# xuhaocuhk/TilinGNN

Measured on AMD Instinct MI355X. Metric: scored tile-nodes/sec (GNN forward), higher is better.
Workload: dtype f32; 1 GPU; TilinGNN.forward on a seeded banded super-graph: 100000 nodes / 1000000 adjacency edges / 1250000 collision edges per GPU, tile_count 2, T=13 edge types, width 32, depth 20, train-mode BatchNorm, graph prep included; n_nodes=100000, n_adj_edges=1000000, n_col_edges=1250000, parallelism=single GPU

## Files before the change

### tilingnn_amd/csrc/graph_prep.hip

```cpp
#include <atomic>
#include <chrono>
#include <mutex>
#include <vector>

#include "tgnn_common.h"

namespace tgnn {

constexpr int kScanThreads = 256;
constexpr int kScanItems = 8;
constexpr int kScanTile = kScanThreads * kScanItems;

__device__ __forceinline__ int wave_inclusive_scan(int v) {
    const int lane = threadIdx.x & 63;
#pragma unroll
    for (int d = 1; d < 64; d <<= 1) {
        int t = __shfl_up(v, d, 64);
        if (lane >= d) v += t;
    }
    return v;
}

__global__ __launch_bounds__(kScanThreads) void scan_tiles_kernel(const int *in, int *out,
                                                                  int *__restrict__ block_sums, int64_t n) {
// ... 894 lines not shown
                        e0 = rpA[row];
                        e1 = rpA[row + 1];
                    }
                    for (int e = e0; e < e1; e += 8) {
                        int ty[8];
#pragma unroll
                        for (int u = 0; u < 8; ++u) ty[u] = e + u < e1 ? A.adj_type[e + u] : -1;
#pragma unroll
                        for (int u = 0; u < 8; ++u)
                            if (ty[u] >= 0) cnt[tid * ld + ty[u]]++;
                    }
                }
                __syncthreads();
                if (act)
                    for (int t = i; t < n_types; t += 16) {
                        int m = 0;
                        for (int r = 0; r < 16; ++r) m = max(m, cnt[(k * 16 + r) * ld + t]);
                        maxm[k * kMaxColTypes + t] = m;
                    }
                __syncthreads();
                if (act && i == 0) {
                    int acc = 0;
                    for (int t = 0; t < n_types; ++t) {
                        base[k * (kMaxColTypes + 1) + t] = acc;
                        acc += maxm[k * kMaxColTypes + t];
                    }
                    base[k * (kMaxColTypes + 1) + n_types] = acc;
                    if (!fill && tile < nt16) g_tile_cols[tile] = acc + 1;
                }
                __syncthreads();
                if (fill && act && tile < nt16) {
                    const int64_t c0 = tile_ptr[tile];
                    const int n_edge_cols = base[k * (kMaxColTypes + 1) + n_types];
                    for (int c = 0; c < n_edge_cols; ++c) A.col_slot_src[(c0 + c) * 16 + i] = -1;
                    for (int t = i; t < n_types; t += 16) {
                        const int m = maxm[k * kMaxColTypes + t];
                        for (int r = 0; r < m; ++r)
                            A.col_meta[c0 + base[k * (kMaxColTypes + 1) + t] + r] = t | (r == 0 ? 1 << 8 : 0) | (r == m - 1 ? 1 << 9 : 0);
                    }
                    const int deg = e1 - e0;
                    A.col_slot_src[(c0 + n_edge_cols) * 16 + i] = row < n ? __float_as_int((float)(deg > 0 ? deg : 1)) : -1;
                    if (i == 0) A.col_meta[c0 + n_edge_cols] = n_types | (1 << 8) | (1 << 9) | (1 << 10);
                    __builtin_amdgcn_fence(__ATOMIC_RELEASE, "wavefront");
                    __builtin_amdgcn_wave_barrier();
                    for (int t = 0; t < n_types; ++t) cnt[tid * ld + t] = 0;
                    for (int e = e0; e < e1; e += 8) {
                        int ty[8], sr[8];
#pragma unroll
                        for (int u = 0; u < 8; ++u) {
                            ty[u] = e + u < e1 ? A.adj_type[e + u] : -1;
                            sr[u] = e + u < e1 ? A.adj_src[e + u] : 0;
                        }
#pragma unroll
                        for (int u = 0; u < 8; ++u)
                            if (ty[u] >= 0) {
                                const int r = cnt[tid * ld + ty[u]]++;
                                A.col_slot_src[(c0 + base[k * (kMaxColTypes + 1) + ty[u]] + r) * 16 + i] = sr[u];
                            }
                    }
                }
                __syncthreads();
            }
            if (!fill) {
                small_prep_barrier(A.ctr, target, G);
                for (int t = tid; t <= nt16; t += NT) tile_ptr[t] = t < nt16 ? g_tile_cols[t] : 0;
                __syncthreads();
                small_block_scan(tile_ptr, nt16 + 1, wave_tot);
                if (blk == 0)
                    for (int t = tid; t <= nt16; t += NT) A.tile_col_ptr[t] = tile_ptr[t];
                __syncthreads();
            }
        }
    } else {
        small_prep_barrier(A.ctr, target, G);
    }
    TGNN_PT
    if (blk == 0 && tid == 0) {
        A.result[0] = n_types;
        A.result[1] = g_flags[0];
        A.result[2] = g_flags[1];
        A.result[3] = ec_valid;
        A.result[4] = maxdeg;
        A.result[5] = cols ? 1 : 0;
        A.result[6] = fallback ? 1 : 0;
        if (!kUnion && A.result_host) {
            const int w[7] = {n_types, g_flags[0], g_flags[1], ec_valid, maxdeg, cols ? 1 : 0, fallback ? 1 : 0};
#pragma unroll
            for (int k = 0; k < 7; ++k) __hip_atomic_store(A.result_host + k, w[k], __ATOMIC_RELAXED, __HIP_MEMORY_SCOPE_SYSTEM);
            for (int k = 7; k < 31; ++k) __hip_atomic_store(A.result_host + k, 0, __ATOMIC_RELAXED, __HIP_MEMORY_SCOPE_SYSTEM);
            __threadfence_system();
            __hip_atomic_store(A.result_host + 31, kPrepWordsMagic, __ATOMIC_RELEASE, __HIP_MEMORY_SCOPE_SYSTEM);
        }
    }
    if (kUnion && blk == 0 && tid >= 7 && tid < 32) A.result[tid] = 0;
    __syncthreads();
    if (tid == 0 && atomicAdd(&A.ctr[1], 1u) == (unsigned)G - 1) {
        __hip_atomic_store(&A.ctr[0], 0u, __ATOMIC_RELAXED, __HIP_MEMORY_SCOPE_AGENT);
        __hip_atomic_store(&A.ctr[1], 0u, __ATOMIC_RELAXED, __HIP_MEMORY_SCOPE_AGENT);
    }
}

__global__ __launch_bounds__(kSmallPrepThreads) void graph_prep_small_kernel(SmallPrepArgs A) {
    graph_prep_small_body<false>(A, (int)blockIdx.x, (int)gridDim.x);
}

__global__ __launch_bounds__(kSmallPrepThreads) void graph_prep_small_union_kernel(const SmallPrepArgs *__restrict__ tab,
                                                                                   const int *__restrict__ first_block, int n_layouts) {
    int lo = 0, hi = n_layouts;
    while (hi - lo > 1) {
        const int mid = (lo + hi) >> 1;
        if (first_block[mid] <= (int)blockIdx.x) lo = mid; else hi = mid;
    }
    const int j = __builtin_amdgcn_readfirstlane(lo);
    const int b0 = __builtin_amdgcn_readfirstlane(first_block[j]), b1 = __builtin_amdgcn_readfirstlane(first_block[j + 1]);
    const SmallPrepArgs *e = tab + j;
    SmallPrepArgs A;
    A.adj_ei = e->adj_ei; A.col_ei = e->col_ei; A.attr = e->attr;
    A.n = e->n; A.ea = e->ea; A.ec = e->ec; A.fe = e->fe; A.max_col_types = e->max_col_types;
    A.adj_rowptr = e->adj_rowptr; A.adj_src = e->adj_src; A.adj_eid = e->adj_eid; A.adj_type = e->adj_type;
    A.edge_type = e->edge_type; A.type_rep = e->type_rep;
    A.col_rowptr = e->col_rowptr; A.col_src = e->col_src; A.col_eid = e->col_eid;
    A.tile_col_ptr = e->tile_col_ptr; A.col_meta = e->col_meta; A.col_slot_src = e->col_slot_src;
    A.result_host = nullptr; A.tmp = e->tmp; A.result = e->result; A.ctr = e->ctr;
    graph_prep_small_body<true>(A, (int)blockIdx.x - b0, b1 - b0);
}

static inline unsigned grid_for(int64_t n, int threads = 256, int cap = 256 * 16) {
    int64_t g = (n + threads - 1) / threads;
    if (g < 1) g = 1;
    if (g > cap) g = cap;
    return (unsigned)g;
}

static inline uint32_t dedup_table_size(int64_t e) {
    uint64_t want = (uint64_t)(e > 512 ? e : 512) * 2;
    uint32_t cap = 1024;
    while (cap < want) cap <<= 1;
    return cap;
}


constexpr int kBkLogMax = 9, kBkRows = 1 << kBkLogMax, kBkMaxBuckets = 4096, kBkThreads = 1024;
constexpr int kBkCap = 15360;
constexpr int kBkCapHalf = 7168;
struct BkSet {
    const int64_t *ei;
    int64_t e;
    int drop_self;
    int *rowptr, *col_src, *col_eid, *err_flag;
    int *rec_eid, *rec_src;
    unsigned short *rec_row;
    int *total_out, *max_deg_out;
};
struct BkArgs {
    BkSet set[2];
    int64_t n, n_src;
    int nb, nblk;
    int lg;
    int cap;
    int cap_lds;
    int *hist;
    const int *tile_off;
    unsigned *scan_ticket;
};
__device__ __forceinline__ int bk_scanned(const BkArgs &A, int64_t i) {
    const int v = A.hist[i];
    return A.tile_off ? v + A.tile_off[i / kScanTile] : v;
}

__global__ __launch_bounds__(kBkThreads) void bk_hist_kernel(BkArgs A) {
    extern __shared__ int bk_h[];
    const BkSet S = A.set[blockIdx.y];
    const int tid = threadIdx.x, blk = blockIdx.x;
    for (int b = tid; b < A.nb; b += kBkThreads) bk_h[b] = 0;
    __syncthreads();
    const int64_t i0 = S.e * blk / A.nblk, i1 = S.e * (blk + 1) / A.nblk;
    for (int64_t i = i0 + tid; i < i1; i += kBkThreads) {
        const int64_t s = S.ei[i], d = S.ei[S.e + i];
        if (s < 0 || s >= A.n_src || d < 0 || d >= A.n) {
            if (S.err_flag) *S.err_flag = 1;
        } else if (!(S.drop_self && s == d)) {
            atomicAdd(&bk_h[d >> A.lg], 1);
        }
    }
    __syncthreads();
    for (int b = tid; b < A.nb; b += kBkThreads) A.hist[((int64_t)blockIdx.y * A.nb + b) * A.nblk + blk] = bk_h[b];
    if (blk == 0 && blockIdx.y == 1 && tid == 0) {
        A.hist[(int64_t)2 * A.nb * A.nblk] = 0;
        if (A.scan_ticket) *A.scan_ticket = 0u;
    }
}

constexpr int kBkChunk = kBkThreads * 8;
__global__ __launch_bounds__(kBkThreads) void bk_scatter_kernel(BkArgs A) {
    extern __shared__ int bk_h[];
    int *cur = bk_h, *lcnt = cur + A.nb, *lstart = lcnt + A.nb, *wtot = lstart + A.nb;
    int *l_eid = wtot + 16, *l_src = l_eid + kBkChunk;
    unsigned short *l_row = reinterpret_cast<unsigned short *>(l_src + kBkChunk), *l_bkt = l_row + kBkChunk;
    const BkSet S = A.set[blockIdx.y];
    const int tid = threadIdx.x, blk = blockIdx.x;
    const int base = bk_scanned(A, (int64_t)blockIdx.y * A.nb * A.nblk);
    for (int b = tid; b < A.nb; b += kBkThreads) cur[b] = bk_scanned(A, ((int64_t)blockIdx.y * A.nb + b) * A.nblk + blk) - base;
    const int64_t i0 = S.e * blk / A.nblk, i1 = S.e * (blk + 1) / A.nblk;
    const int per = (A.nb + kBkThreads - 1) / kBkThreads;
    for (int64_t c0 = i0; c0 < i1; c0 += kBkChunk) {
        for (int b = tid; b < A.nb; b += kBkThreads) lcnt[b] = 0;
        __syncthreads();
        int e_b[8], e_r[8], e_s[8], e_row[8];
#pragma unroll
        for (int u = 0; u < 8; ++u) {
            const int64_t i = c0 + tid + (int64_t)u * kBkThreads;
            e_b[u] = -1;
            if (i < i1) {
                const int64_t sv = S.ei[i], d = S.ei[S.e + i];
                if (!(sv < 0 || sv >= A.n_src || d < 0 || d >= A.n || (S.drop_self && sv == d))) {
                    e_b[u] = (int)(d >> A.lg);
                    e_row[u] = (int)(d & ((1 << A.lg) - 1));
                    e_s[u] = (int)sv;
                    e_r[u] = atomicAdd(&lcnt[e_b[u]], 1);
                }
            }
        }
        __syncthreads();
        {
            int mine = 0;
            for (int q = 0; q < per; ++q) {
                const int b = tid * per + q;
                mine += b < A.nb ? lcnt[b] : 0;
            }
            const int incl = wave_inclusive_scan(mine);
            if ((tid & 63) == 63) wtot[tid >> 6] = incl;
            __syncthreads();
            int run = incl - mine;
            for (int w = 0; w < (tid >> 6); ++w) run += wtot[w];
            for (int q = 0; q < per; ++q) {
                const int b = tid * per + q;
                if (b < A.nb) {
                    lstart[b] = run;
                    run += lcnt[b];
                }
            }
        }
        __syncthreads();
        int total = 0;
#pragma unroll
        for (int u = 0; u < 8; ++u)
            if (e_b[u] >= 0) {
                const int at = lstart[e_b[u]] + e_r[u];
                l_eid[at] = (int)(c0 + tid + (int64_t)u * kBkThreads);
                l_src[at] = e_s[u];
                l_row[at] = (unsigned short)e_row[u];
                l_bkt[at] = (unsigned short)e_b[u];
            }
        total = lstart[A.nb - 1] + lcnt[A.nb - 1];
        __syncthreads();
        for (int j = tid; j < total; j += kBkThreads) {
            const int b = l_bkt[j];
            const int g = cur[b] + (j - lstart[b]);
            S.rec_eid[g] = l_eid[j];
            S.rec_src[g] = l_src[j];
            S.rec_row[g] = l_row[j];
        }
        __syncthreads();
        for (int b = tid; b < A.nb; b += kBkThreads) cur[b] += lcnt[b];
    }
}

__global__ __launch_bounds__(kBkThreads) void bk_rows_kernel(BkArgs A) {
    extern __shared__ int bk_l[];
    const int rows = 1 << A.lg;
    int *cnt = bk_l, *off = bk_l + rows, *wtot = off + rows + 1, *key_s = wtot + 16, *val_s = key_s + A.cap_lds;
    unsigned short *row_s = reinterpret_cast<unsigned short *>(val_s + A.cap_lds);
    const BkSet S = A.set[blockIdx.y];
    const int tid = threadIdx.x, b = blockIdx.x;
    const int base = bk_scanned(A, (int64_t)blockIdx.y * A.nb * A.nblk);
    const int lo = bk_scanned(A, ((int64_t)blockIdx.y * A.nb + b) * A.nblk) - base;
    const int hi = bk_scanned(A, ((int64_t)blockIdx.y * A.nb + b + 1) * A.nblk) - base;
    const int m = hi - lo;
    const bool in_lds = m <= A.cap;
    if (tid < rows) cnt[tid] = 0;
    __syncthreads();
    if (in_lds) {
        for (int j = tid; j < m; j += kBkThreads) atomicAdd(&cnt[S.rec_row[lo + j]], 1);
    } else if (tid < rows) {
        int c = 0;
        for (int j = 0; j < m; ++j) c += S.rec_row[lo + j] == tid ? 1 : 0;
        cnt[tid] = c;
    }
    __syncthreads();
    int mine = 0, incl = 0;
    if (tid < rows) {
        mine = cnt[tid];
        incl = wave_inclusive_scan(mine);
        if ((tid & 63) == 63) wtot[tid >> 6] = incl;
    }
    __syncthreads();
    if (tid < rows) {
        int woff = 0;
        for (int w = 0; w < (tid >> 6); ++w) woff += wtot[w];
        off[tid] = woff + incl - mine;
        if (tid == rows - 1) off[rows] = woff + incl;
        const int64_t row = (int64_t)b * rows + tid;
        if (row < A.n) S.rowptr[row] = lo + off[tid];
        cnt[tid] = 0;
    }
    if (b == A.nb - 1 && tid == 0) {
        S.rowptr[A.n] = hi;
        if (S.total_out) *S.total_out = hi;
    }
    if (S.max_deg_out && tid < rows) {
        int md = mine;
#pragma unroll
        for (int d = 32; d >= 1; d >>= 1) md = max(md, __shfl_xor(md, d, 64));
        if ((tid & 63) == 0) wtot[8 + (tid >> 6)] = md;
    }
    __syncthreads();
    if (S.max_deg_out && tid == 0) {
        int md = 0;
        for (int w = 0; w < (rows >> 6); ++w) md = max(md, wtot[8 + w]);
        if (md > 0) atomicMax(S.max_deg_out, md);
    }
    if (in_lds) {
        for (int j = tid; j < m; j += kBkThreads) {
            const int r = S.rec_row[lo + j];
            const int at = off[r] + atomicAdd(&cnt[r], 1);
            key_s[at] = S.rec_eid[lo + j];
            val_s[at] = S.rec_src[lo + j];
            row_s[at] = (unsigned short)r;
        }
        __syncthreads();
        for (int j = tid; j < m; j += kBkThreads) {
            const int r = row_s[j], rb = off[r], re = off[r + 1], key = key_s[j];
            int rank = 0;
            for (int q = rb; q < re; ++q) rank += key_s[q] < key ? 1 : 0;
            S.col_eid[lo + rb + rank] = key;
            S.col_src[lo + rb + rank] = val_s[j];
        }
    } else if (tid < rows) {
        int *ke = S.col_eid + lo + off[tid], *ks = S.col_src + lo + off[tid];
        int c = 0;
        for (int j = 0; j < m; ++j)
            if (S.rec_row[lo + j] == tid) {
                ke[c] = S.rec_eid[lo + j];
                ks[c] = S.rec_src[lo + j];
                ++c;
            }
        for (int i = 1; i < c; ++i) {
            const int key = ke[i], val = ks[i];
            int j = i - 1;
            while (j >= 0 && ke[j] > key) {
                ke[j + 1] = ke[j];
                ks[j + 1] = ks[j];
                --j;
            }
            ke[j + 1] = key;
            ks[j + 1] = val;
        }
    }
}

static std::atomic<int> g_bk_cap{kBkCap};
static int prep_side_stream(hipStream_t *st, hipEvent_t *fork, hipEvent_t *join) {
    static std::mutex mu;
    static hipStream_t streams[64] = {};
    static thread_local hipEvent_t events[64][2] = {};
    int dev = 0;
    if (hipGetDevice(&dev) != hipSuccess || dev < 0 || dev >= 64) return TGNN_ERR_INVALID_ARG;
    {
        std::lock_guard<std::mutex> lock(mu);
        if (!streams[dev] && hipStreamCreateWithFlags(&streams[dev], hipStreamNonBlocking) != hipSuccess) return TGNN_ERR_INVALID_ARG;
    }
    if (!events[dev][0])
        for (int k = 0; k < 2; ++k)
            if (hipEventCreateWithFlags(&events[dev][k], hipEventDisableTiming) != hipSuccess) return TGNN_ERR_INVALID_ARG;
    *st = streams[dev];
    *fork = events[dev][0];
    *join = events[dev][1];
    return TGNN_OK;
}

static thread_local hipEvent_t g_prep_words_ev[64] = {};
static hipError_t prep_words_event(hipEvent_t *ev) {
    int dev = 0;
    hipError_t e = hipGetDevice(&dev);
    if (e != hipSuccess) return e;
    if (dev < 0 || dev >= 64) return hipErrorInvalidDevice;
    if (!g_prep_words_ev[dev]) {
        e = hipEventCreateWithFlags(&g_prep_words_ev[dev], hipEventDisableTiming);
        if (e != hipSuccess) return e;
    }
    *ev = g_prep_words_ev[dev];
    return hipSuccess;
}

static thread_local volatile int32_t *g_prep_poll[64] = {};
static std::atomic<int> g_prep_poll_on{1};

extern "C" int32_t tgnn_set_prep_words_poll(int32_t on) {
    if (on < 0) return g_prep_poll_on.load();
    return g_prep_poll_on.exchange(on ? 1 : 0);
}

extern "C" int tgnn_graph_prep_wait(tgnn_stream_t stream) {
    DeviceGuard guard__(stream);
    int dev = 0;
    TGNN_CHECK_HIP(hipGetDevice(&dev));
    if (dev >= 0 && dev < 64 && g_prep_poll[dev]) {
        volatile int32_t *h = g_prep_poll[dev];
        g_prep_poll[dev] = nullptr;
        const auto t0 = std::chrono::steady_clock::now();
        for (unsigned spins = 0;; ++spins) {
            if (__atomic_load_n(const_cast<const int32_t *>(h) + 31, __ATOMIC_ACQUIRE) == kPrepWordsMagic) return TGNN_OK;
            __builtin_ia32_pause();
            if ((spins & 1023) == 1023 && std::chrono::steady_clock::now() - t0 > std::chrono::seconds(2)) break;
        }
        TGNN_CHECK_HIP(hipStreamSynchronize(static_cast<hipStream_t>(stream)));
        if (__atomic_load_n(const_cast<const int32_t *>(h) + 31, __ATOMIC_ACQUIRE) == kPrepWordsMagic) return TGNN_OK;
        set_error("tgnn_graph_prep_wait: the result words never reached the host buffer");
        return TGNN_ERR_INVALID_ARG;
    }
    hipEvent_t ev = nullptr;
    TGNN_CHECK_HIP(prep_words_event(&ev));
    TGNN_CHECK_HIP(hipEventSynchronize(ev));
    return TGNN_OK;
}

static int bk_blocks(int64_t e_max) {
    int64_t nblk = (e_max + 8191) / 8192;
    return (int)(nblk < 1 ? 1 : (nblk > 256 ? 256 : nblk));
}
static int bk_log_rows(int64_t n, int64_t e_max) {
    return (n <= (int64_t)256 * kBkMaxBuckets && e_max * 256 <= (int64_t)3584 * (n > 0 ? n : 1)) ? 8 : 9;
}
static size_t bk_workspace_bytes(int64_t n, int64_t ea, int64_t ec) {
    const int64_t rows = (int64_t)1 << bk_log_rows(n, ea > ec ? ea : ec);
    const int64_t nb = (n + rows - 1) / rows, nblk = bk_blocks(ea > ec ? ea : ec), cells = 2 * nb * nblk + 1;
    return align_up((size_t)cells * 4, 256) + scan_ws_ints(cells) * 4 + align_up((size_t)(ea > 0 ? ea : 1) * 10, 256) +
           align_up((size_t)(ec > 0 ? ec : 1) * 10, 256) + 2048;
}
static bool bk_fits(int64_t n) { return (n + kBkRows - 1) / kBkRows <= kBkMaxBuckets; }

static int csr_build_pair_bucketed(const int64_t *adj_ei, int64_t ea, const int64_t *col_ei, int64_t ec, int64_t n, int64_t n_src,
                                   int *a_rowptr, int *a_src, int *a_eid, int *a_err, int *c_rowptr, int *c_src, int *c_eid,
                                   int *c_err, int *a_max_deg, int *c_total, void *ws, size_t ws_bytes, hipStream_t s) {
    BkArgs A{};
    A.n = n; A.n_src = n_src;
    A.lg = bk_log_rows(n, ea > ec ? ea : ec);
    A.nb = (int)((n + ((int64_t)1 << A.lg) - 1) >> A.lg);
    A.nblk = bk_blocks(ea > ec ? ea : ec);
    A.cap_lds = A.lg == 8 ? kBkCapHalf : kBkCap;
    A.cap = g_bk_cap.load() < A.cap_lds ? g_bk_cap.load() : A.cap_lds;
    const int64_t cells = (int64_t)2 * A.nb * A.nblk + 1;
    Carver cv(ws, ws_bytes);
    A.hist = cv.take<int>(cells);
    int *scan_ws = cv.take<int>(scan_ws_ints(cells));
    const int64_t es[2] = {ea, ec};
    for (int k = 0; k < 2; ++k) {
        const int64_t e1 = es[k] > 0 ? es[k] : 1;
        unsigned char *rec = cv.take<unsigned char>((size_t)e1 * 10);
        A.set[k].rec_eid = reinterpret_cast<int *>(rec);
        A.set[k].rec_src = reinterpret_cast<int *>(rec + (size_t)e1 * 4);
        A.set[k].rec_row = reinterpret_cast<unsigned short *>(rec + (size_t)e1 * 8);
    }
    A.set[0].ei = adj_ei; A.set[0].e = ea; A.set[0].drop_self = 0;
    A.set[0].rowptr = a_rowptr; A.set[0].col_src = a_src; A.set[0].col_eid = a_eid; A.set[0].err_flag = a_err;
    A.set[1].ei = col_ei; A.set[1].e = ec; A.set[1].drop_self = 1;
    A.set[1].rowptr = c_rowptr; A.set[1].col_src = c_src; A.set[1].col_eid = c_eid; A.set[1].err_flag = c_err;
    A.set[0].max_deg_out = a_max_deg;
    A.set[1].total_out = c_total;
    const size_t lds_h = (size_t)A.nb * sizeof(int);
    const int64_t scan_tiles = (cells + kScanTile - 1) / kScanTile;
    const bool fused_scan = cells > kScanOneMax && scan_tiles <= kScanFusedTiles;
    if (fused_scan) {
        A.tile_off = scan_ws + align_up((size_t)scan_tiles, 64);
        A.scan_ticket = reinterpret_cast<unsigned *>(scan_ws + scan_ws_ints(cells) - 32);
    }
    bk_hist_kernel<<<dim3(A.nblk, 2), kBkThreads, lds_h, s>>>(A);
    if (fused_scan)
        scan_tiles_fused_kernel<<<(unsigned)scan_tiles, kScanThreads, 0, s>>>(A.hist, A.hist, scan_ws, const_cast<int *>(A.tile_off), cells,
                                                                             A.scan_ticket);
    else
        exclusive_scan_i32(A.hist, A.hist, cells, scan_ws, s);
    const size_t lds_s = (size_t)(3 * A.nb + 16 + 2 * kBkChunk) * sizeof(int) + (size_t)2 * kBkChunk * sizeof(unsigned short);
    static LdsOptIn site_s;
    TGNN_CHECK_HIP(opt_in_dynamic_lds(bk_scatter_kernel, (int)(160 * 1024 - 256), site_s));
    bk_scatter_kernel<<<dim3(A.nblk, 2), kBkThreads, lds_s, s>>>(A);
    const size_t lds_r = (size_t)(2 * (1 << A.lg) + 1 + 16 + 2 * A.cap_lds) * sizeof(int) + (size_t)A.cap_lds * sizeof(unsigned short);
    static LdsOptIn site;
    TGNN_CHECK_HIP(opt_in_dynamic_lds(bk_rows_kernel, (int)(160 * 1024 - 256), site));
    bk_rows_kernel<<<dim3(A.nb, 2), kBkThreads, lds_r, s>>>(A);
    TGNN_CHECK_LAUNCH();
    return TGNN_OK;
}

}

using namespace tgnn;

#ifdef TGNN_DEBUG
extern "C" int32_t tgnn_debug_set_csr_bucket_cap(int32_t cap) {
    const int prev = g_bk_cap.load();
    if (cap >= 0) g_bk_cap.store(cap > kBkCap ? kBkCap : cap);
    return prev;
}
#endif

extern "C" size_t tgnn_csr_workspace_bytes(int64_t n_nodes, int64_t n_edges) {
    return align_up((size_t)(n_nodes + 1) * 4, 256) + align_up((size_t)(n_edges > 0 ? n_edges : 1) * 4, 256) +
           scan_ws_ints(n_nodes + 1) * 4 + 1024;
}

extern "C" int tgnn_csr_build(const int64_t *edge_index, int64_t n_edges, int64_t n_nodes, int64_t n_src_nodes,
                              int drop_self_loops, int32_t *rowptr, int32_t *col_src, int32_t *col_eid, int32_t *err_flag, void *ws,
                              size_t ws_bytes, tgnn_stream_t stream) {
    DeviceGuard guard__(stream);
    TGNN_CHECK_ARG(n_nodes >= 0 && n_nodes < (1ll << 31) - 1, "n_nodes must fit int32");
    TGNN_CHECK_ARG(n_src_nodes >= n_nodes && n_src_nodes < (1ll << 31) - 1, "n_src_nodes must be >= n_nodes and fit int32");
    TGNN_CHECK_ARG(n_edges >= 0 && n_edges < (1ll << 31) - 1, "n_edges must fit int32");
    TGNN_CHECK_ARG(rowptr && (n_edges == 0 || (edge_index && col_src && col_eid)), "null pointer");
    if (ws_bytes < tgnn_csr_workspace_bytes(n_nodes, n_edges) || !ws) {
        set_error("tgnn_csr_build: workspace too small");
        return TGNN_ERR_WORKSPACE;
    }
    hipStream_t s = static_cast<hipStream_t>(stream);
    Carver cv(ws, ws_bytes);
    int *cnt = cv.take<int>(n_nodes + 1);
    int *rank = cv.take<int>(n_edges > 0 ? n_edges : 1);
    int *scan_ws = cv.take<int>(scan_ws_ints(n_nodes + 1));
    TGNN_CHECK_HIP(hipMemsetAsync(cnt, 0, (size_t)(n_nodes + 1) * 4, s));
    if (n_edges > 0)
        csr_count_kernel<<<grid_for(n_edges), 256, 0, s>>>(edge_index, n_edges, n_nodes, n_src_nodes, drop_self_loops, cnt,
                                                           rank, err_flag);
    exclusive_scan_i32(cnt, rowptr, n_nodes + 1, scan_ws, s);
    if (n_edges > 0) {
        csr_fill_kernel<<<grid_for(n_edges), 256, 0, s>>>(edge_index, n_edges, rowptr, rank, col_src, col_eid);
        csr_sort_rows_kernel<<<(unsigned)((n_nodes + kSortRows - 1) / kSortRows), kSortRows, 0, s>>>(rowptr, n_nodes, col_src,
                                                                                                  col_eid);
    }
    TGNN_CHECK_LAUNCH();
    return TGNN_OK;
}

extern "C" size_t tgnn_edge_dedup_workspace_bytes(int64_t n_edges, int32_t fe) {
    (void)fe;
    return (size_t)dedup_table_size(n_edges) * 4 + align_up((size_t)n_edges * 4, 256) * 2 +
           scan_ws_ints(n_edges) * 4 + 2048 + (size_t)(kDedupListMax + 64) * 4 + 512;
}

static int edge_type_dedup_listed(const float *edge_attr, int64_t n_edges, int32_t fe, int32_t *edge_type, int32_t *type_rep_edge,
                                  int32_t *n_types, int32_t *fallback, void *ws, size_t ws_bytes, hipStream_t s) {
    (void)ws_bytes;
    Carver cv(ws, ws_bytes);
    const uint32_t cap = dedup_table_size(n_edges);
    int *table = cv.take<int>(cap + 64);
    int *slot_of_edge = cv.take<int>(n_edges);
    int *first_rank = cv.take<int>(n_edges);
    int *rep_slots = cv.take<int>(kDedupListMax);
    TGNN_CHECK_HIP(hipMemsetAsync(table, 0xFF, (size_t)(cap + 64) * 4, s));
    if (fe <= 60)
        dedup_insert_kernel<<<grid_for(n_edges, kDedupRows), kDedupRows, (size_t)kDedupRows * (fe | 1) * 4, s>>>(
            edge_attr, n_edges, fe, table, cap - 1, slot_of_edge, table + cap, rep_slots);
    else
        dedup_insert_direct_kernel<<<grid_for(n_edges), 256, 0, s>>>(edge_attr, n_edges, fe, table, cap - 1, slot_of_edge, table + cap,
                                                                     rep_slots);
    dedup_rank_kernel<<<1, 1024, 0, s>>>(table, table + cap, rep_slots, first_rank, type_rep_edge, n_types, fallback);
    dedup_assign_kernel<<<grid_for(n_edges), 256, 0, s>>>(table, slot_of_edge, first_rank, n_edges, edge_type, type_rep_edge,
                                                          nullptr, fallback);
    TGNN_CHECK_LAUNCH();
    return TGNN_OK;
}

extern "C" int tgnn_edge_type_dedup(const float *edge_attr, int64_t n_edges, int32_t fe, int32_t *edge_type,
                                    int32_t *type_rep_edge, int32_t *n_types, void *ws, size_t ws_bytes,
                                    tgnn_stream_t stream) {
    DeviceGuard guard__(stream);
    TGNN_CHECK_ARG(n_edges >= 0 && n_edges < (1ll << 30), "n_edges out of range");
    TGNN_CHECK_ARG(fe >= 1, "fe must be >= 1");
    TGNN_CHECK_ARG(n_types, "null n_types");
    hipStream_t s = static_cast<hipStream_t>(stream);
    if (n_edges == 0) {
        TGNN_CHECK_HIP(hipMemsetAsync(n_types, 0, 4, s));
        return TGNN_OK;
    }
    TGNN_CHECK_ARG(edge_attr && edge_type && type_rep_edge, "null pointer");
    if (ws_bytes < tgnn_edge_dedup_workspace_bytes(n_edges, fe) || !ws) {
        set_error("tgnn_edge_type_dedup: workspace too small");
        return TGNN_ERR_WORKSPACE;
    }
    Carver cv(ws, ws_bytes);
    const uint32_t cap = dedup_table_size(n_edges);
    int *table = cv.take<int>(cap);
    int *slot_of_edge = cv.take<int>(n_edges);
    int *is_first = cv.take<int>(n_edges);
    int *scan_ws = cv.take<int>(scan_ws_ints(n_edges));
    TGNN_CHECK_HIP(hipMemsetAsync(table, 0xFF, (size_t)cap * 4, s));
    if (fe <= 60)
        dedup_insert_kernel<<<grid_for(n_edges, kDedupRows), kDedupRows, (size_t)kDedupRows * (fe | 1) * 4, s>>>(
            edge_attr, n_edges, fe, table, cap - 1, slot_of_edge);
    else
        dedup_insert_direct_kernel<<<grid_for(n_edges), 256, 0, s>>>(edge_attr, n_edges, fe, table, cap - 1, slot_of_edge);
    dedup_mark_first_kernel<<<grid_for(n_edges), 256, 0, s>>>(table, slot_of_edge, n_edges, is_first);
    exclusive_scan_i32(is_first, is_first, n_edges, scan_ws, s);
    dedup_assign_kernel<<<grid_for(n_edges), 256, 0, s>>>(table, slot_of_edge, is_first, n_edges, edge_type,
                                                          type_rep_edge, n_types);
    TGNN_CHECK_LAUNCH();
    return TGNN_OK;
}

extern "C" int tgnn_gather_i32(const int32_t *src, int64_t n_src, const int32_t *idx, int64_t n, int32_t *out,
                               tgnn_stream_t stream) {
    DeviceGuard guard__(stream);
    if (n <= 0) return TGNN_OK;
    TGNN_CHECK_ARG(src && idx && out, "null pointer");
    gather_i32_kernel<<<grid_for(n), 256, 0, static_cast<hipStream_t>(stream)>>>(src, n_src, idx, n, out);
    TGNN_CHECK_LAUNCH();
    return TGNN_OK;
}

extern "C" int64_t tgnn_nnconv_cols_max_columns(int64_t n_nodes, int64_t n_edges) {
    return n_edges + (n_nodes + kColTileRows - 1) / kColTileRows + 32;
}

extern "C" size_t tgnn_nnconv_cols_workspace_bytes(int64_t n_nodes) {
    const int64_t ntiles = (n_nodes + kColTileRows - 1) / kColTileRows;
    return align_up((size_t)(ntiles + 1) * 4, 256) + scan_ws_ints(ntiles + 1) * 4 + 1024;
}

extern "C" int tgnn_nnconv_cols_build(const int32_t *rowptr, const int32_t *col_src, const int32_t *col_type,
                                      int64_t n_nodes, int32_t n_types, int32_t *tile_col_ptr, int32_t *col_meta,
                                      int32_t *col_slot_src, void *ws, size_t ws_bytes, tgnn_stream_t stream) {
    DeviceGuard guard__(stream);
    TGNN_CHECK_ARG(n_nodes >= 1, "n_nodes");
    TGNN_CHECK_ARG(n_types >= 0 && n_types <= kMaxColTypes, "the column NNConv structure supports at most 40 edge types");
    TGNN_CHECK_ARG(rowptr && tile_col_ptr && col_meta && col_slot_src, "null pointer");
    TGNN_CHECK_ARG(n_types == 0 || (col_src && col_type), "null CSR pointer");
    if (!ws || ws_bytes < tgnn_nnconv_cols_workspace_bytes(n_nodes)) {
        set_error("tgnn_nnconv_cols_build: workspace too small");
        return TGNN_ERR_WORKSPACE;
    }
    hipStream_t s = static_cast<hipStream_t>(stream);
    const int64_t nt16 = (n_nodes + kColTileRows - 1) / kColTileRows;
    Carver cv(ws, ws_bytes);
// ... 374 lines not shown
        if (u.host) (void)hipHostFree(u.host);
        u.host = nullptr;
        u.host_cap = 0;
        TGNN_CHECK_HIP(hipHostMalloc(reinterpret_cast<void **>(&u.host), tab_bytes * 2, hipHostMallocDefault));
        u.host_cap = tab_bytes * 2;
    }
    unsigned *ctr = reinterpret_cast<unsigned *>(u.dev);
    char *tab_dev = u.dev + ctr_bytes;
    SmallPrepArgs *args = reinterpret_cast<SmallPrepArgs *>(u.host);
    int *fb = reinterpret_cast<int *>(u.host + arg_bytes);
    const SmallPrepArgs *args_dev = reinterpret_cast<const SmallPrepArgs *>(tab_dev);
    const int *fb_dev = reinterpret_cast<const int *>(tab_dev + arg_bytes);
    struct Group { int first, count, blocks, fb_at; };
    std::vector<Group> groups((size_t)n_groups, Group{0, 0, 0, 0});
    const int max_col_types = tgnn_nnconv_cols_max_types();
    int fb_at = 0;
    for (int j = 0; j < k; ++j) {
        const tgnn_small_prep_layout &l = layouts[j];
        SmallPrepArgs A{};
        A.adj_ei = l.adj_edge_index; A.col_ei = l.col_edge_index; A.attr = l.adj_edge_attr;
        A.n = l.n_nodes; A.ea = l.n_adj_edges; A.ec = l.n_col_edges; A.fe = l.fe;
        A.max_col_types = max_col_types;
        A.adj_rowptr = l.adj_rowptr; A.adj_src = l.adj_src; A.adj_eid = l.adj_eid; A.adj_type = l.adj_type;
        A.edge_type = l.edge_type; A.type_rep = l.type_rep_edge;
        A.col_rowptr = l.col_rowptr; A.col_src = l.col_src; A.col_eid = l.col_eid;
        A.tile_col_ptr = l.tile_col_ptr; A.col_meta = l.col_meta; A.col_slot_src = l.col_slot_src;
        A.tmp = l.tmp;
        A.result = results_dev + (size_t)j * 32;
        A.ctr = ctr + (size_t)j * 32;
        args[j] = A;
        Group &G = groups[(size_t)group[(size_t)j]];
        if (G.count == 0) {
            G.first = j;
            G.fb_at = fb_at++;
            fb[G.fb_at] = 0;
        }
        G.blocks += blocks[(size_t)j];
        G.count += 1;
        fb[fb_at++] = G.blocks;
    }
    TGNN_CHECK_HIP(hipMemcpyAsync(tab_dev, u.host, tab_bytes, hipMemcpyHostToDevice, s));
    int rc = TGNN_OK;
    int64_t launched = 0, prepared = 0;
    for (const Group &G : groups) {
        if (hipMemsetAsync(ctr + (size_t)G.first * 32, 0, (size_t)G.count * 128, s) != hipSuccess) {
            set_error("tgnn_graph_prep_small_many: hipMemsetAsync of the counters failed");
            rc = TGNN_ERR_LAUNCH;
            break;
        }
        struct Ctx { const SmallPrepArgs *tab; const int *fb; int count, blocks; } ctx{args_dev + G.first, fb_dev + G.fb_at, G.count, G.blocks};
        rc = spin_kernel_chain(s, [](void *c, hipStream_t st) {
            Ctx *x = static_cast<Ctx *>(c);
            graph_prep_small_union_kernel<<<dim3(x->blocks), dim3(kSmallPrepThreads), kSmallPrepLds, st>>>(x->tab, x->fb, x->count);
        }, &ctx, G.blocks);
        if (rc != TGNN_OK) break;
        ++launched;
        prepared += G.count;
    }
    if (rc == TGNN_OK && hipMemcpyAsync(results_host, results_dev, (size_t)k * 32 * sizeof(int32_t), hipMemcpyDeviceToHost, s) != hipSuccess) {
        set_error("tgnn_graph_prep_small_many: the copy of the result words could not be queued");
        rc = TGNN_ERR_LAUNCH;
    }
    (void)hipEventRecord(ev_words, s);
    (void)hipEventRecord(u.ev, s);
    g_prep_many_count[0].fetch_add(launched, std::memory_order_relaxed);
    g_prep_many_count[1].fetch_add(prepared, std::memory_order_relaxed);
    if (rc != TGNN_OK) return rc;
    TGNN_CHECK_LAUNCH();
    return TGNN_OK;
}

extern "C" int tgnn_graph_prep_small_many_wait(tgnn_stream_t stream) {
    DeviceGuard guard__(stream);
    hipEvent_t ev = nullptr;
    TGNN_CHECK_HIP(prep_many_event(&ev));
    TGNN_CHECK_HIP(hipEventSynchronize(ev));
    return TGNN_OK;
}

__global__ __launch_bounds__(256) void prep_result_kernel(const int *__restrict__ col_rowptr, const int *__restrict__ adj_rowptr,
                                                          int64_t n, int *__restrict__ result) {
    if (blockIdx.x == 0 && threadIdx.x == 0) result[3] = col_rowptr[n];
    int md = 0;
    for (int64_t r = (int64_t)blockIdx.x * 256 + threadIdx.x; r < n; r += (int64_t)gridDim.x * 256)
        md = max(md, adj_rowptr[r + 1] - adj_rowptr[r]);
#pragma unroll
    for (int d = 32; d >= 1; d >>= 1) md = max(md, __shfl_xor(md, d, 64));
    __shared__ int wm[4];
    if ((threadIdx.x & 63) == 0) wm[threadIdx.x >> 6] = md;
    __syncthreads();
    if (threadIdx.x == 0) atomicMax(result + 4, max(max(wm[0], wm[1]), max(wm[2], wm[3])));
}

extern "C" size_t tgnn_graph_prep_workspace_bytes(int64_t n_nodes, int64_t n_adj_edges, int64_t n_col_edges, int32_t fe) {
    const int64_t emax = n_adj_edges > n_col_edges ? n_adj_edges : n_col_edges;
    return align_up(tgnn_csr_workspace_bytes(n_nodes, emax), 256) + align_up(bk_workspace_bytes(n_nodes, n_adj_edges, n_col_edges), 256) +
           align_up(tgnn_edge_dedup_workspace_bytes(n_adj_edges, fe), 256) +
           align_up(tgnn_nnconv_cols_workspace_bytes(n_nodes), 256) + 1024;
}

extern "C" int tgnn_graph_prep(const int64_t *adj_edge_index, int64_t n_adj_edges, const float *adj_edge_attr, int32_t fe,
                               const int64_t *col_edge_index, int64_t n_col_edges, int64_t n_nodes, int64_t n_src_nodes,
                               int32_t *adj_rowptr, int32_t *adj_src, int32_t *adj_eid, int32_t *adj_type, int32_t *edge_type,
                               int32_t *type_rep_edge,
                               int32_t *col_rowptr, int32_t *col_src, int32_t *col_eid, int32_t *tile_col_ptr, int32_t *col_meta,
                               int32_t *col_slot_src, int32_t *mid_tile_nb, uint32_t *mid_ent, int32_t *tile_grp_ptr, int32_t *grp,
                               void *ws, size_t ws_bytes, int32_t *result, int32_t *result_host, tgnn_stream_t stream) {
    DeviceGuard guard__(stream);
    TGNN_CHECK_ARG(n_nodes >= 1 && fe >= 1 && n_adj_edges >= 0 && n_col_edges >= 0, "shape");
    TGNN_CHECK_ARG(n_src_nodes >= n_nodes && n_src_nodes < (1ll << 31) - 1, "n_src_nodes must be >= n_nodes and fit int32");
    const bool want_cols = tile_col_ptr != nullptr, want_eg = tile_grp_ptr != nullptr;
    TGNN_CHECK_ARG(adj_rowptr && col_rowptr && result, "null pointer");
    TGNN_CHECK_ARG(want_cols || want_eg, "no NNConv structure asked for (type columns and / or edge groups)");
    TGNN_CHECK_ARG(!want_cols || (col_meta && col_slot_src), "type columns: tile_col_ptr, col_meta, col_slot_src go together");
    TGNN_CHECK_ARG(!want_eg || (grp && ((uintptr_t)grp % 8) == 0), "edge groups: tile_grp_ptr and an 8-byte aligned grp go together");
    TGNN_CHECK_ARG(want_cols || !(mid_tile_nb && mid_ent), "the mid-size batches are built from the type columns");
    if (!ws || ws_bytes < tgnn_graph_prep_workspace_bytes(n_nodes, n_adj_edges, n_col_edges, fe)) {
        set_error("tgnn_graph_prep: workspace too small");
        return TGNN_ERR_WORKSPACE;
    }
    hipStream_t s = static_cast<hipStream_t>(stream);
    const int64_t emax = n_adj_edges > n_col_edges ? n_adj_edges : n_col_edges;
    Carver cv(ws, ws_bytes);
    const size_t csr_b = tgnn_csr_workspace_bytes(n_nodes, emax), dd_b = tgnn_edge_dedup_workspace_bytes(n_adj_edges, fe),
                 col_b = tgnn_nnconv_cols_workspace_bytes(n_nodes);
    void *ws_csr = cv.take<unsigned char>(csr_b), *ws_dd = cv.take<unsigned char>(dd_b), *ws_col = cv.take<unsigned char>(col_b);
    TGNN_CHECK_HIP(hipMemsetAsync(result, 0, 32 * sizeof(int32_t), s));
    hipStream_t s_side = nullptr;
    hipEvent_t ev_fork = nullptr, ev_join = nullptr;
    if (n_adj_edges > 0 && prep_side_stream(&s_side, &ev_fork, &ev_join) == TGNN_OK) {
        TGNN_CHECK_HIP(hipEventRecord(ev_fork, s));
        TGNN_CHECK_HIP(hipStreamWaitEvent(s_side, ev_fork, 0));
    } else {
        s_side = nullptr;
    }
    int rc;
    bool bucketed = false;
    auto bail = [&](int code) {
        if (s_side && hipEventRecord(ev_join, s_side) == hipSuccess) (void)hipStreamWaitEvent(s, ev_join, 0);
        return code;
    };
    const bool csr_first = n_adj_edges + n_col_edges >= 1000000;
    auto queue_dedup = [&]() -> int {
        if (!s_side) return TGNN_OK;
        rc = edge_type_dedup_listed(adj_edge_attr, n_adj_edges, fe, edge_type, type_rep_edge, result + 0, result + 6, ws_dd, dd_b, s_side);
        if (rc != TGNN_OK) return bail(rc);
        if (hipEventRecord(ev_join, s_side) != hipSuccess) {
            (void)hipStreamSynchronize(s_side);
            set_error("tgnn_graph_prep: hipEventRecord failed");
            return TGNN_ERR_LAUNCH;
        }
        return TGNN_OK;
    };
    if (!csr_first) {
        const int rcd = queue_dedup();
        if (rcd != TGNN_OK) return rcd;
    }
    if (bk_fits(n_nodes) && n_adj_edges < (int64_t(1) << 31) - 1 && n_col_edges < (int64_t(1) << 31) - 1) {
        const size_t bk_b = bk_workspace_bytes(n_nodes, n_adj_edges, n_col_edges);
        void *ws_bk = cv.take<unsigned char>(bk_b);
        rc = csr_build_pair_bucketed(adj_edge_index, n_adj_edges, col_edge_index, n_col_edges, n_nodes, n_src_nodes, adj_rowptr, adj_src,
                                     adj_eid, result + 1, col_rowptr, col_src, col_eid, result + 2, result + 4, result + 3, ws_bk, bk_b, s);
        if (rc != TGNN_OK) return bail(rc);
        bucketed = true;
    } else {
        rc = tgnn_csr_build(adj_edge_index, n_adj_edges, n_nodes, n_src_nodes, 0, adj_rowptr, adj_src, adj_eid, result + 1, ws_csr, csr_b, stream);
        if (rc != TGNN_OK) return bail(rc);
        rc = tgnn_csr_build(col_edge_index, n_col_edges, n_nodes, n_src_nodes, 1, col_rowptr, col_src, col_eid, result + 2, ws_csr, csr_b, stream);
        if (rc != TGNN_OK) return bail(rc);
    }
    if (csr_first) {
        const int rcd = queue_dedup();
        if (rcd != TGNN_OK) return rcd;
    }
    if (s_side) {
        TGNN_CHECK_HIP(hipStreamWaitEvent(s, ev_join, 0));
    } else {
        rc = tgnn_edge_type_dedup(adj_edge_attr, n_adj_edges, fe, edge_type, type_rep_edge, result + 0, ws_dd, dd_b, stream);
        if (rc != TGNN_OK) return rc;
    }
    if (!bucketed) {
        int64_t rb = (n_nodes + 1023) / 1024;
        prep_result_kernel<<<(unsigned)(rb > 256 ? 256 : rb), 256, 0, s>>>(col_rowptr, adj_rowptr, n_nodes, result);
    }
    int32_t *host_words_dev = nullptr;
    if (result_host && want_eg && !want_cols && !(mid_tile_nb && mid_ent) && g_prep_poll_on.load(std::memory_order_relaxed)) {
        int dev = 0;
        void *dptr = nullptr;
        if (hipGetDevice(&dev) == hipSuccess && dev >= 0 && dev < 64 && hipHostGetDevicePointer(&dptr, result_host, 0) == hipSuccess && dptr) {
            if (g_prep_poll[dev]) TGNN_CHECK_HIP(hipDeviceSynchronize());
            host_words_dev = static_cast<int32_t *>(dptr);
            __atomic_store_n(result_host + 31, 0, __ATOMIC_RELEASE);
            g_prep_poll[dev] = result_host;
        } else {
            (void)hipGetLastError();
        }
    }
    if (result_host && !host_words_dev) {
        hipEvent_t ev_words = nullptr;
        TGNN_CHECK_HIP(prep_words_event(&ev_words));
        if (s_side) {
            TGNN_CHECK_HIP(hipEventRecord(ev_fork, s));
            TGNN_CHECK_HIP(hipStreamWaitEvent(s_side, ev_fork, 0));
            TGNN_CHECK_HIP(hipMemcpyAsync(result_host, result, 32 * sizeof(int32_t), hipMemcpyDeviceToHost, s_side));
            TGNN_CHECK_HIP(hipEventRecord(ev_words, s_side));
        } else {
            TGNN_CHECK_HIP(hipMemcpyAsync(result_host, result, 32 * sizeof(int32_t), hipMemcpyDeviceToHost, s));
            TGNN_CHECK_HIP(hipEventRecord(ev_words, s));
        }
    }
    const int64_t nt16 = (n_nodes + kColTileRows - 1) / kColTileRows;
    Carver cc(ws_col, col_b);
    int *tile_cols = cc.take<int>(nt16 + 1);
    int *scan_ws = cc.take<int>(scan_ws_ints(nt16 + 1));
    const unsigned blocks = (unsigned)((n_nodes + 63) / 64);
    const int max_types = tgnn_nnconv_cols_max_types();
    if (want_cols) {
        nnconv_col_kernel<false><<<blocks, 64, 0, s>>>(adj_rowptr, adj_src, adj_type, n_nodes, 0, tile_cols, nullptr, nullptr, nullptr,
                                                       result + 0, max_types, nullptr, n_adj_edges > 0 ? edge_type : nullptr, adj_eid,
                                                       n_adj_edges > 0 ? adj_type : nullptr);
        exclusive_scan_i32(tile_cols, tile_col_ptr, nt16 + 1, scan_ws, s);
        nnconv_col_kernel<true><<<blocks, 64, 0, s>>>(adj_rowptr, adj_src, adj_type, n_nodes, 0, nullptr, tile_col_ptr, col_meta,
                                                      col_slot_src, result + 0, max_types, result + 5);
    }
    if (want_eg) {
        const bool gather_types = !want_cols && n_adj_edges > 0;
        launch_nnconv_eg_build(adj_rowptr, adj_src, adj_type, n_nodes, 0, result + 0, max_types, tile_cols, tile_grp_ptr, grp, scan_ws,
                               result + 10, s, gather_types ? edge_type : nullptr, gather_types ? adj_eid : nullptr,
                               host_words_dev ? result : nullptr, host_words_dev);
    }
    TGNN_CHECK_LAUNCH();
    if (mid_tile_nb && mid_ent) {
        rc = tgnn_mid_entries_build(tile_col_ptr, col_meta, col_slot_src, n_nodes, result + 5, mid_tile_nb, mid_ent, result + 8, stream);
        if (rc != TGNN_OK) return rc;
    }
    return TGNN_OK;
}
```

Baseline: 54.60 million nodes/s.

## Fuse edge-group counting and tile scan into bucketed CSR rows kernel

The bucketed CSR row-sort kernel now also gathers each adjacency edge's type and counts per-tile, per-type groups in LDS. The last block to finish, chosen by an atomic ticket, runs a global exclusive scan over tile group counts and publishes the host result words. The separate count and scan passes of the edge-group build are dropped, leaving only the fill kernel. The join with the dedup side stream moves to just before the rows kernel. In exchange the rows kernel needs more LDS, carries extra per-edge work, and relies on a single-block serial scan plus last-block synchronisation.

```diff
diff --git a/tilingnn_amd/csrc/graph_prep.hip b/tilingnn_amd/csrc/graph_prep.hip
--- a/tilingnn_amd/csrc/graph_prep.hip
+++ b/tilingnn_amd/csrc/graph_prep.hip
@@ -1070,6 +1070,17 @@
     unsigned short *rec_row;
     int *total_out, *max_deg_out;
 };
+struct BkEg {
+    const int *edge_type;
+    int *col_type;
+    const int *n_types_dev;
+    int max_types;
+    int *tile_grp_ptr;
+    int *built_flag;
+    const int *result_words;
+    int *host_words;
+    unsigned *ticket;
+};
 struct BkArgs {
     BkSet set[2];
     int64_t n, n_src;
@@ -1080,6 +1091,7 @@
     int *hist;
     const int *tile_off;
     unsigned *scan_ticket;
+    BkEg eg;
 };
 __device__ __forceinline__ int bk_scanned(const BkArgs &A, int64_t i) {
     const int v = A.hist[i];
@@ -1106,6 +1118,7 @@
     if (blk == 0 && blockIdx.y == 1 && tid == 0) {
         A.hist[(int64_t)2 * A.nb * A.nblk] = 0;
         if (A.scan_ticket) *A.scan_ticket = 0u;
+        if (A.eg.ticket) *A.eg.ticket = 0u;
     }
 }
 
@@ -1189,8 +1202,16 @@
     const int rows = 1 << A.lg;
     int *cnt = bk_l, *off = bk_l + rows, *wtot = off + rows + 1, *key_s = wtot + 16, *val_s = key_s + A.cap_lds;
     unsigned short *row_s = reinterpret_cast<unsigned short *>(val_s + A.cap_lds);
+    int *tcnt = reinterpret_cast<int *>(row_s + A.cap_lds);
     const BkSet S = A.set[blockIdx.y];
     const int tid = threadIdx.x, b = blockIdx.x;
+    const bool eg = A.eg.tile_grp_ptr != nullptr, eg_rows = eg && blockIdx.y == 0;
+    bool eg_ok = false;
+    if (eg_rows) {
+        const int n_types = *A.eg.n_types_dev;
+        eg_ok = n_types <= A.eg.max_types && n_types <= kMaxColTypes;
+        for (int j = tid; j < (rows >> 4) * (kMaxColTypes + 1); j += kBkThreads) tcnt[j] = 0;
+    }
     const int base = bk_scanned(A, (int64_t)blockIdx.y * A.nb * A.nblk);
     const int lo = bk_scanned(A, ((int64_t)blockIdx.y * A.nb + b) * A.nblk) - base;
     const int hi = bk_scanned(A, ((int64_t)blockIdx.y * A.nb + b + 1) * A.nblk) - base;
@@ -1224,7 +1245,7 @@
     }
     if (b == A.nb - 1 && tid == 0) {
         S.rowptr[A.n] = hi;
-        if (S.total_out) *S.total_out = hi;
+        if (S.total_out) __hip_atomic_store(S.total_out, hi, __ATOMIC_RELAXED, __HIP_MEMORY_SCOPE_AGENT);
     }
     if (S.max_deg_out && tid < rows) {
         int md = mine;
@@ -1253,6 +1274,11 @@
             for (int q = rb; q < re; ++q) rank += key_s[q] < key ? 1 : 0;
             S.col_eid[lo + rb + rank] = key;
             S.col_src[lo + rb + rank] = val_s[j];
+            if (eg_rows) {
+                const int t = A.eg.edge_type[key];
+                A.eg.col_type[lo + rb + rank] = t;
+                if (eg_ok && (unsigned)t < (unsigned)kMaxColTypes) atomicAdd(&tcnt[(r >> 4) * (kMaxColTypes + 1) + t], 1);
+            }
         }
     } else if (tid < rows) {
         int *ke = S.col_eid + lo + off[tid], *ks = S.col_src + lo + off[tid];
@@ -1274,6 +1300,61 @@
             ke[j + 1] = key;
             ks[j + 1] = val;
         }
+        if (eg_rows)
+            for (int i = 0; i < c; ++i) {
+                const int t = A.eg.edge_type[ke[i]];
+                A.eg.col_type[lo + off[tid] + i] = t;
+                if (eg_ok && (unsigned)t < (unsigned)kMaxColTypes) atomicAdd(&tcnt[(tid >> 4) * (kMaxColTypes + 1) + t], 1);
+            }
+    }
+    if (!eg) return;
+    __syncthreads();
+    const int64_t n_tiles = (A.n + kColTileRows - 1) / kColTileRows;
+    if (eg_rows && tid < (rows >> 4)) {
+        const int64_t tile = (int64_t)b * (rows >> 4) + tid;
+        if (tile < n_tiles) {
+            int g = 0;
+            if (eg_ok) {
+                g = 1;
+                for (int t = 0; t < kMaxColTypes; ++t) g += (tcnt[tid * (kMaxColTypes + 1) + t] + 15) >> 4;
+            }
+            __hip_atomic_store(A.eg.tile_grp_ptr + tile, g, __ATOMIC_RELAXED, __HIP_MEMORY_SCOPE_AGENT);
+        }
+    }
+    __threadfence();
+    __syncthreads();
+    if (tid == 0) {
+        __threadfence();
+        wtot[0] = (int)__hip_atomic_fetch_add(A.eg.ticket, 1u, __ATOMIC_RELAXED, __HIP_MEMORY_SCOPE_AGENT);
+    }
+    __syncthreads();
+    if ((unsigned)wtot[0] != gridDim.x * gridDim.y - 1) return;
+    __threadfence();
+    if (A.eg.host_words && tid < 32) {
+        const int v = __hip_atomic_load(A.eg.result_words + tid, __ATOMIC_RELAXED, __HIP_MEMORY_SCOPE_AGENT);
+        if (tid < 31) __hip_atomic_store(A.eg.host_words + tid, v, __ATOMIC_RELAXED, __HIP_MEMORY_SCOPE_SYSTEM);
+        __threadfence_system();
+        if (tid == 31) __hip_atomic_store(A.eg.host_words + 31, kPrepWordsMagic, __ATOMIC_RELEASE, __HIP_MEMORY_SCOPE_SYSTEM);
+    }
+    if (tid == 0) {
+        if (A.eg.built_flag && *A.eg.n_types_dev <= A.eg.max_types && *A.eg.n_types_dev <= kMaxColTypes) *A.eg.built_flag = 1;
+        __hip_atomic_store(A.eg.ticket, 0u, __ATOMIC_RELAXED, __HIP_MEMORY_SCOPE_AGENT);
+    }
+    __syncthreads();
+    const int64_t m1 = n_tiles + 1, per = (m1 + kBkThreads - 1) / kBkThreads;
+    const int64_t i0 = tid * per, i1 = i0 + per < m1 ? i0 + per : m1;
+    int sum = 0;
+    for (int64_t i = i0; i < i1; ++i)
+        sum += i < n_tiles ? __hip_atomic_load(A.eg.tile_grp_ptr + i, __ATOMIC_RELAXED, __HIP_MEMORY_SCOPE_AGENT) : 0;
+    const int incl2 = wave_inclusive_scan(sum);
+    if ((tid & 63) == 63) wtot[tid >> 6] = incl2;
+    __syncthreads();
+    int run = incl2 - sum;
+    for (int w = 0; w < (tid >> 6); ++w) run += wtot[w];
+    for (int64_t i = i0; i < i1; ++i) {
+        const int x = i < n_tiles ? __hip_atomic_load(A.eg.tile_grp_ptr + i, __ATOMIC_RELAXED, __HIP_MEMORY_SCOPE_AGENT) : 0;
+        A.eg.tile_grp_ptr[i] = run;
+        run += x;
     }
 }
 
@@ -1358,9 +1439,11 @@
 }
 static bool bk_fits(int64_t n) { return (n + kBkRows - 1) / kBkRows <= kBkMaxBuckets; }
 
+template <class F>
 static int csr_build_pair_bucketed(const int64_t *adj_ei, int64_t ea, const int64_t *col_ei, int64_t ec, int64_t n, int64_t n_src,
                                    int *a_rowptr, int *a_src, int *a_eid, int *a_err, int *c_rowptr, int *c_src, int *c_eid,
-                                   int *c_err, int *a_max_deg, int *c_total, void *ws, size_t ws_bytes, hipStream_t s) {
+                                   int *c_err, int *a_max_deg, int *c_total, void *ws, size_t ws_bytes, hipStream_t s,
+                                   const BkEg *eg, F &&before_rows) {
     BkArgs A{};
     A.n = n; A.n_src = n_src;
     A.lg = bk_log_rows(n, ea > ec ? ea : ec);
@@ -1393,6 +1476,10 @@
         A.tile_off = scan_ws + align_up((size_t)scan_tiles, 64);
         A.scan_ticket = reinterpret_cast<unsigned *>(scan_ws + scan_ws_ints(cells) - 32);
     }
+    if (eg) {
+        A.eg = *eg;
+        A.eg.ticket = reinterpret_cast<unsigned *>(scan_ws + scan_ws_ints(cells) - 31);
+    }
     bk_hist_kernel<<<dim3(A.nblk, 2), kBkThreads, lds_h, s>>>(A);
     if (fused_scan)
         scan_tiles_fused_kernel<<<(unsigned)scan_tiles, kScanThreads, 0, s>>>(A.hist, A.hist, scan_ws, const_cast<int *>(A.tile_off), cells,
@@ -1403,9 +1490,12 @@
     static LdsOptIn site_s;
     TGNN_CHECK_HIP(opt_in_dynamic_lds(bk_scatter_kernel, (int)(160 * 1024 - 256), site_s));
     bk_scatter_kernel<<<dim3(A.nblk, 2), kBkThreads, lds_s, s>>>(A);
-    const size_t lds_r = (size_t)(2 * (1 << A.lg) + 1 + 16 + 2 * A.cap_lds) * sizeof(int) + (size_t)A.cap_lds * sizeof(unsigned short);
+    const size_t lds_r = (size_t)(2 * (1 << A.lg) + 1 + 16 + 2 * A.cap_lds) * sizeof(int) + (size_t)A.cap_lds * sizeof(unsigned short) +
+                         (eg ? (size_t)((1 << A.lg) >> 4) * (kMaxColTypes + 1) * sizeof(int) : 0);
     static LdsOptIn site;
     TGNN_CHECK_HIP(opt_in_dynamic_lds(bk_rows_kernel, (int)(160 * 1024 - 256), site));
+    const int rc_join = before_rows();
+    if (rc_join != TGNN_OK) return rc_join;
     bk_rows_kernel<<<dim3(A.nb, 2), kBkThreads, lds_r, s>>>(A);
     TGNN_CHECK_LAUNCH();
     return TGNN_OK;
@@ -2086,37 +2176,6 @@
         }
         return TGNN_OK;
     };
-    if (!csr_first) {
-        const int rcd = queue_dedup();
-        if (rcd != TGNN_OK) return rcd;
-    }
-    if (bk_fits(n_nodes) && n_adj_edges < (int64_t(1) << 31) - 1 && n_col_edges < (int64_t(1) << 31) - 1) {
-        const size_t bk_b = bk_workspace_bytes(n_nodes, n_adj_edges, n_col_edges);
-        void *ws_bk = cv.take<unsigned char>(bk_b);
-        rc = csr_build_pair_bucketed(adj_edge_index, n_adj_edges, col_edge_index, n_col_edges, n_nodes, n_src_nodes, adj_rowptr, adj_src,
-                                     adj_eid, result + 1, col_rowptr, col_src, col_eid, result + 2, result + 4, result + 3, ws_bk, bk_b, s);
-        if (rc != TGNN_OK) return bail(rc);
-        bucketed = true;
-    } else {
-        rc = tgnn_csr_build(adj_edge_index, n_adj_edges, n_nodes, n_src_nodes, 0, adj_rowptr, adj_src, adj_eid, result + 1, ws_csr, csr_b, stream);
-        if (rc != TGNN_OK) return bail(rc);
-        rc = tgnn_csr_build(col_edge_index, n_col_edges, n_nodes, n_src_nodes, 1, col_rowptr, col_src, col_eid, result + 2, ws_csr, csr_b, stream);
-        if (rc != TGNN_OK) return bail(rc);
-    }
-    if (csr_first) {
-        const int rcd = queue_dedup();
-        if (rcd != TGNN_OK) return rcd;
-    }
-    if (s_side) {
-        TGNN_CHECK_HIP(hipStreamWaitEvent(s, ev_join, 0));
-    } else {
-        rc = tgnn_edge_type_dedup(adj_edge_attr, n_adj_edges, fe, edge_type, type_rep_edge, result + 0, ws_dd, dd_b, stream);
-        if (rc != TGNN_OK) return rc;
-    }
-    if (!bucketed) {
-        int64_t rb = (n_nodes + 1023) / 1024;
-        prep_result_kernel<<<(unsigned)(rb > 256 ? 256 : rb), 256, 0, s>>>(col_rowptr, adj_rowptr, n_nodes, result);
-    }
     int32_t *host_words_dev = nullptr;
     if (result_host && want_eg && !want_cols && !(mid_tile_nb && mid_ent) && g_prep_poll_on.load(std::memory_order_relaxed)) {
         int dev = 0;
@@ -2130,6 +2189,61 @@
             (void)hipGetLastError();
         }
     }
+    const int max_types = tgnn_nnconv_cols_max_types();
+    bool dedup_queued = false, joined = false;
+    if (!csr_first) {
+        const int rcd = queue_dedup();
+        if (rcd != TGNN_OK) return rcd;
+        dedup_queued = true;
+    }
+    bool fused_eg = false;
+    if (bk_fits(n_nodes) && n_adj_edges < (int64_t(1) << 31) - 1 && n_col_edges < (int64_t(1) << 31) - 1) {
+        const size_t bk_b = bk_workspace_bytes(n_nodes, n_adj_edges, n_col_edges);
+        void *ws_bk = cv.take<unsigned char>(bk_b);
+        fused_eg = want_eg && !want_cols && s_side && adj_type && edge_type;
+        BkEg eg{};
+        if (fused_eg) {
+            eg.edge_type = edge_type; eg.col_type = adj_type;
+            eg.n_types_dev = result + 0; eg.max_types = max_types;
+            eg.tile_grp_ptr = tile_grp_ptr; eg.built_flag = result + 10;
+            eg.result_words = host_words_dev ? result : nullptr; eg.host_words = host_words_dev;
+        }
+        auto before_rows = [&]() -> int {
+            if (!fused_eg) return TGNN_OK;
+            if (!dedup_queued) {
+                const int rcd = queue_dedup();
+                if (rcd != TGNN_OK) return rcd;
+                dedup_queued = true;
+            }
+            TGNN_CHECK_HIP(hipStreamWaitEvent(s, ev_join, 0));
+            joined = true;
+            return TGNN_OK;
+        };
+        rc = csr_build_pair_bucketed(adj_edge_index, n_adj_edges, col_edge_index, n_col_edges, n_nodes, n_src_nodes, adj_rowptr, adj_src,
+                                     adj_eid, result + 1, col_rowptr, col_src, col_eid, result + 2, result + 4, result + 3, ws_bk, bk_b, s,
+                                     fused_eg ? &eg : nullptr, before_rows);
+        if (rc != TGNN_OK) return bail(rc);
+        bucketed = true;
+    } else {
+        rc = tgnn_csr_build(adj_edge_index, n_adj_edges, n_nodes, n_src_nodes, 0, adj_rowptr, adj_src, adj_eid, result + 1, ws_csr, csr_b, stream);
+        if (rc != TGNN_OK) return bail(rc);
+        rc = tgnn_csr_build(col_edge_index, n_col_edges, n_nodes, n_src_nodes, 1, col_rowptr, col_src, col_eid, result + 2, ws_csr, csr_b, stream);
+        if (rc != TGNN_OK) return bail(rc);
+    }
+    if (!dedup_queued) {
+        const int rcd = queue_dedup();
+        if (rcd != TGNN_OK) return rcd;
+    }
+    if (s_side) {
+        if (!joined) TGNN_CHECK_HIP(hipStreamWaitEvent(s, ev_join, 0));
+    } else {
+        rc = tgnn_edge_type_dedup(adj_edge_attr, n_adj_edges, fe, edge_type, type_rep_edge, result + 0, ws_dd, dd_b, stream);
+        if (rc != TGNN_OK) return rc;
+    }
+    if (!bucketed) {
+        int64_t rb = (n_nodes + 1023) / 1024;
+        prep_result_kernel<<<(unsigned)(rb > 256 ? 256 : rb), 256, 0, s>>>(col_rowptr, adj_rowptr, n_nodes, result);
+    }
     if (result_host && !host_words_dev) {
         hipEvent_t ev_words = nullptr;
         TGNN_CHECK_HIP(prep_words_event(&ev_words));
@@ -2148,7 +2262,6 @@
     int *tile_cols = cc.take<int>(nt16 + 1);
     int *scan_ws = cc.take<int>(scan_ws_ints(nt16 + 1));
     const unsigned blocks = (unsigned)((n_nodes + 63) / 64);
-    const int max_types = tgnn_nnconv_cols_max_types();
     if (want_cols) {
         nnconv_col_kernel<false><<<blocks, 64, 0, s>>>(adj_rowptr, adj_src, adj_type, n_nodes, 0, tile_cols, nullptr, nullptr, nullptr,
                                                        result + 0, max_types, nullptr, n_adj_edges > 0 ? edge_type : nullptr, adj_eid,
@@ -2157,7 +2270,10 @@
         nnconv_col_kernel<true><<<blocks, 64, 0, s>>>(adj_rowptr, adj_src, adj_type, n_nodes, 0, nullptr, tile_col_ptr, col_meta,
                                                       col_slot_src, result + 0, max_types, result + 5);
     }
-    if (want_eg) {
+    if (want_eg && fused_eg) {
+        nnconv_eg_kernel<true><<<blocks, 64, 0, s>>>(adj_rowptr, adj_src, adj_type, n_nodes, 0, nullptr, tile_grp_ptr,
+                                                     reinterpret_cast<int2 *>(grp), result + 0, max_types, nullptr);
+    } else if (want_eg) {
         const bool gather_types = !want_cols && n_adj_edges > 0;
         launch_nnconv_eg_build(adj_rowptr, adj_src, adj_type, n_nodes, 0, result + 0, max_types, tile_cols, tile_grp_ptr, grp, scan_ws,
                                result + 10, s, gather_types ? edge_type : nullptr, gather_types ? adj_eid : nullptr,
```

New measurement: 47.40 million nodes/s. 13.2% lower.
